# violetamenendez/zest-nerf

Hardware: AMD Instinct MI355X
Metric: rendered rays/sec (1024-ray x 128-sample batch per GPU) (higher is better)
Workload: dtype bf16; 1 GPU; nsff_static_1024x128; rays_per_gpu=1024, samples_per_ray=128, rays_total=1024, collective=none, ranks=1, backend=none

## Files before the change

### zest-nerf_amd/build_hip.py

```python
import os
import subprocess
import sys
from concurrent.futures import ThreadPoolExecutor

HERE = os.path.dirname(os.path.abspath(__file__))
CSRC = os.path.join(HERE, "csrc")
OBJ = os.path.join(CSRC, "build")
LIB = os.path.join(HERE, "libzest_hip.so")
SOURCES = ["capi.hip", "composite.hip", "composite_bwd.hip", "encode.hip", "rays.hip", "volume_cost.hip", "costreg.hip", "losses.hip", "mlp_plan.hip", "mlp.hip", "mlp_engine.hip", "mlp_train.hip", "mlp_train16.hip",
           "mlp_train16_dw.hip", "fused.hip"]
SOURCE_FLAGS = {"mlp_engine.hip": ["-fno-slp-vectorize"], "mlp_train16.hip": ["-fno-slp-vectorize"]}
_SHAPES = [("s4d2", 4, "true", 2, "false"), ("s2d2", 2, "true", 2, "false"), ("s4d0", 4, "true", 0, "false"),
           ("s2d0", 2, "true", 0, "false"), ("s0d0", 0, "true", 0, "false"), ("s4", 4, "false", 0, "false"),
           ("s2", 2, "false", 0, "false"), ("s0", 0, "false", 0, "false"),
           ("s4v", 4, "false", 0, "true"), ("s2v", 2, "false", 0, "true")]
_PRECS = [("x3", "ZEST_PREC_F16X3"), ("bf16", "ZEST_PREC_BF16"), ("f16", "ZEST_PREC_F16")]
VARIANTS = [("fused_%s_%s" % (pt, tag),
             ["-DZEST_V_PTAG=%s" % pt, "-DZEST_V_EP=%s" % ep, "-DZEST_V_TAG=%s" % tag, "-DZEST_V_NTS=%d" % nts,
              "-DZEST_V_DYN=%s" % dyn, "-DZEST_V_NTD=%d" % ntd, "-DZEST_V_V2=%s" % v2] +
             (["-fno-slp-vectorize"] if (nts or ntd) else []) +
             (["-mllvm", "-amdgpu-use-amdgpu-trackers=1"] if ((nts or ntd) and pt != "x3") else []) +
             (["-mllvm", "-amdgpu-sched-strategy=max-ilp"] if tag == "s0" else []))
            for tag, nts, dyn, ntd, v2 in _SHAPES for pt, ep in _PRECS]
HIPCC = os.environ.get("HIPCC", "/opt/rocm/bin/hipcc")
FLAGS = ["-O3", "--offload-arch=gfx950", "-fPIC", "-std=c++17", "-Wall", "-Wno-unused-function",
         "-Wno-inline-asm",
         "-mllvm", "-pragma-unroll-threshold=1000000"]


def _deps():
    hdr = [os.path.join(CSRC, f) for f in os.listdir(CSRC) if f.endswith((".cuh", ".h"))]
    hdr.append(os.path.join(HERE, "..", "include", "zest_render.h"))
    return hdr


def _stale(target, srcs):
    if not os.path.exists(target):
        return True
    t = os.path.getmtime(target)
    return any(os.path.getmtime(s) > t for s in srcs if os.path.exists(s))


def _compile(src, extra, objname=None):
    obj = os.path.join(OBJ, (objname or src.replace(".hip", "")) + ".o")
    path = os.path.join(CSRC, src)
    if _stale(obj, [path] + _deps()):
        cmd = [HIPCC] + FLAGS + extra + ["-Rpass-analysis=kernel-resource-usage", "-c", path, "-o", obj]
        r = subprocess.run(cmd, capture_output=True, text=True)
        if r.returncode != 0:
            raise RuntimeError("hipcc failed for %s:\n%s" % (src, r.stderr[-6000:]))
        remarks = [l for l in r.stderr.splitlines() if "-Rpass-analysis=kernel-resource-usage" in l]
        with open(obj[:-2] + ".remarks", "w") as f:
            f.write("\n".join(remarks) + "\n")
        rest = [l for l in r.stderr.splitlines() if "-Rpass-analysis=kernel-resource-usage" not in l
                and "loop not unrolled" not in l]
        if any(("warning" in l or "error" in l) for l in rest):
            sys.stderr.write("\n".join(rest) + "\n")
    return obj


def build(force=False, extra_flags=(), tag=None, only=None):
    global OBJ, LIB
    if tag:
        OBJ = os.path.join(CSRC, "build_" + tag)
        LIB = os.path.join(HERE, "libzest_hip_%s.so" % tag)
    os.makedirs(OBJ, exist_ok=True)
    every = [(name, "fused_variant.hip", flags) for name, flags in VARIANTS]
    every += [(s.replace(".hip", ""), s, SOURCE_FLAGS.get(s, [])) for s in SOURCES]
    jobs = [j for j in every if not only or j[0] in only or j[1] in only]
    if force:
        for name, _, _ in jobs:
            o = os.path.join(OBJ, name + ".o")
            if os.path.exists(o):
                os.remove(o)
    with ThreadPoolExecutor(max_workers=int(os.environ.get("ZEST_BUILD_JOBS", "8"))) as ex:
        objs = list(ex.map(lambda j: _compile(j[1], j[2] + list(extra_flags), j[0]), jobs))
    default_obj = os.path.join(CSRC, "build")
    objs += [os.path.join(default_obj, j[0] + ".o") for j in every if j not in jobs]
    if _stale(LIB, objs):
        cmd = [HIPCC, "--offload-arch=gfx950", "-shared", "-fPIC", "-o", LIB] + objs + ["-lrocblas"]
        r = subprocess.run(cmd, capture_output=True, text=True)
        if r.returncode != 0:
            raise RuntimeError("link failed:\n" + r.stderr[-4000:])
    return LIB


if __name__ == "__main__":
    argv = sys.argv[1:]
    tag = argv[argv.index("--tag") + 1] if "--tag" in argv else None
    only = argv[argv.index("--only") + 1].split(",") if "--only" in argv else None
    print(build(force="-f" in argv, extra_flags=[a for a in argv if a.startswith("-D")] + [a[7:] for a in argv if a.startswith("--flag=")], tag=tag, only=only))
```

### zest-nerf_amd/csrc/fused.cuh

```cuda
#pragma once
#include "mlp_engine.cuh"
#include "zest_sample_ops.cuh"

namespace zest {

constexpr int kMaxViews = 16;
constexpr int kCamStride = 24;

struct FusedNet {
    const float *bias;
    const uint4 *tiles;
    const float4 *vol;
    const float4 *imgs;
    const float *w2cs, *intr;
    int D, Hv, Wv, V, H, W;
    int head, v2;
};

struct FusedArgs {
    const float *ndc, *pts, *z, *dir;
    int R, S;
    FusedNet st, dy;
    float frame_idx;
    int white_bkgd;
// ... 158 lines not shown
#pragma unroll
        for (int i = 0; i < NK * 8; i++)
            v[i] = __builtin_amdgcn_fractf(ndc[0] * (13.37f + (float)i) + ndc[2] * 7.1f + (float)grp * 0.31f) - 0.25f;
    }
    valid = false;
#endif
    const int rv = feat_volume_round(n.V);
    if (valid) {
        float vv[4] = {0.f, 0.f, 0.f, 0.f};
        if (grp < 2) {
            float fx = zest_unnorm(ndc[0], n.Wv), fy = zest_unnorm(ndc[1], n.Hv), fz = zest_unnorm(ndc[2], n.D);
            fx = fminf(fmaxf(fx, -2.0f), (float)n.Wv + 1.0f);
            fy = fminf(fmaxf(fy, -2.0f), (float)n.Hv + 1.0f);
            fz = fminf(fmaxf(fz, -2.0f), (float)n.D + 1.0f);
            const float x0f = floorf(fx), y0f = floorf(fy), z0f = floorf(fz);
            const float tx = fx - x0f, ty = fy - y0f, tz = fz - z0f;
            const int x0 = (int)x0f, y0 = (int)y0f, z0 = (int)z0f;
            float4 tap[8];
            float wgt[8];
#pragma unroll
            for (int c = 0; c < 8; c++) {
                const int dx = c & 1, dy = (c >> 1) & 1, dz = c >> 2;
                const int xi = x0 + dx, yi = y0 + dy, zi = z0 + dz;
                const bool ok = (unsigned)xi < (unsigned)n.Wv && (unsigned)yi < (unsigned)n.Hv &&
                                (unsigned)zi < (unsigned)n.D;
                const int xc = min(max(xi, 0), n.Wv - 1), yc = min(max(yi, 0), n.Hv - 1),
                          zc = min(max(zi, 0), n.D - 1);
                wgt[c] = ok ? (dx ? tx : 1.0f - tx) * (dy ? ty : 1.0f - ty) * (dz ? tz : 1.0f - tz) : 0.0f;
#ifdef ZEST_EXPERIMENT_TAP_SAME
                tap[c] = n.vol[(((yc * n.Wv + xc) * n.D + zc) & 0) + grp];
#else
                tap[c] = n.vol[2 * ((yc * n.Wv + xc) * n.D + zc) + grp];
#endif
            }
#pragma unroll
            for (int c = 0; c < 8; c++) {
                vv[0] = fmaf(wgt[c], tap[c].x, vv[0]), vv[1] = fmaf(wgt[c], tap[c].y, vv[1]);
                vv[2] = fmaf(wgt[c], tap[c].z, vv[2]), vv[3] = fmaf(wgt[c], tap[c].w, vv[3]);
            }
        }
#pragma unroll
        for (int r = 0; r < 2 * NK; r++) {
            float *dst = v + 8 * (r >> 1) + 4 * (r & 1);
            if (r < rv) {
                view_tap(4 * r + grp, dst);
            } else if (r == rv) {
                if (n.V > 4 * rv) view_tap(grp >= 2 ? 4 * rv + grp - 2 : n.V, dst);
                if (grp < 2) dst[0] = vv[0], dst[1] = vv[1], dst[2] = vv[2], dst[3] = vv[3];
            }
        }
    }
#pragma unroll
    for (int t = 0; t < NK; t++) {
        float w8[8];
#pragma unroll
        for (int e = 0; e < 8; e++) w8[e] = v[8 * t + e];
        store_tile<EP>(w8, op, t);
    }
}

template <bool PROJ>
__device__ __forceinline__ void stage_cams(const FusedNet &n, float *lds) {
    if (!n.w2cs) return;
    const int nv = n.imgs ? n.V : 1;
    for (int i = threadIdx.x; i < nv * kCamStride; i += blockDim.x) {
        const int v = i / kCamStride, k = i % kCamStride;
        float val = 0.0f;
        if constexpr (PROJ) {
            if (k < 12 && n.intr) {
                const int row = k >> 2, col = k & 3;
                const float *K = n.intr + 9 * v + 3 * row, *Rt = n.w2cs + 16 * v + col;
                val = fmaf(K[2], Rt[8], fmaf(K[1], Rt[4], K[0] * Rt[0]));
            } else if (k >= 12) {
                val = n.w2cs[16 * v + (k - 12)];
            }
        } else {
            if (k < 12) val = n.w2cs[16 * v + k];
            else if (k < 21 && n.intr) val = n.intr[9 * v + (k - 12)];
        }
        lds[i] = val;
    }
}

#ifndef ZEST_FUSED_WAVES
#define ZEST_FUSED_WAVES 8
#endif
constexpr int kFusedWaves = ZEST_FUSED_WAVES;
constexpr int kPartialFloats = 20;
constexpr int fused_cb(int EP) { return EP == ZEST_PREC_F16X3 ? 1 : 2; }

struct BlockSamples {
    float x[4], pw[3], zz, dist;
    bool valid;
};

template <int BS>
__device__ __forceinline__ float block_sum(float v) {
    if constexpr (BS == 32) return lower_half_sum(v);
    v += dpp_f<0xB1>(0.f, v);
    v += dpp_f<0x4E>(0.f, v);
    v += dpp_f<0x141>(0.f, v);
    v += dpp_f<0x140>(0.f, v);
    return readlane_f<0>(v);
}
template <int BS>
__device__ __forceinline__ float block_excl_prod(float f, int c, float *total) {
    if constexpr (BS == 32) return lower_half_excl_prod(f, c, total);
    float v = f;
    v *= dpp_f<0x111>(1.f, v);
    v *= dpp_f<0x112>(1.f, v);
    v *= dpp_f<0x114>(1.f, v);
    v *= dpp_f<0x118>(1.f, v);
    *total = readlane_f<15>(v);
    const float ex = dpp_f<0x138>(1.f, v);
    return c == 0 ? 1.0f : ex;
}

#ifndef ZEST_FUSED_WG_PER_CU
#define ZEST_FUSED_WG_PER_CU 1
#endif
#ifndef ZEST_REBUILD_PTS
#define ZEST_REBUILD_PTS 0
#endif
#ifndef ZEST_GATHER_FENCE
#define ZEST_GATHER_FENCE 1
#endif
#ifndef ZEST_EARLY_DYN_GATHER
#define ZEST_EARLY_DYN_GATHER 0
#endif
template <int EP, int NT_FEAT_S, bool DYN, int NT_FEAT_D, bool V2S = false>
__global__ __launch_bounds__(kFusedWaves * 64, kFusedWaves * ZEST_FUSED_WG_PER_CU / 4) void fused_blocks_kernel(FusedArgs a) {
    constexpr bool MOD_S = NT_FEAT_S > 0, MOD_D = NT_FEAT_D > 0;
    constexpr int NP = ep_parts(EP), CB = fused_cb(EP), BS = 16 * CB;
    if constexpr (EP == ZEST_PREC_F16) engine_fp16_overflow_clamp();
    constexpr int UNITS_S = stream_units(4, NT_FEAT_S, NP), UNITS_D = DYN ? stream_units(6, NT_FEAT_D, NP) : 0;
    using Ring = RingTiles<kFusedWaves, UNITS_S, UNITS_D>;
    constexpr int kFdBytes = (DYN && MOD_D && ZEST_EARLY_DYN_GATHER) ? kFusedWaves * CB * (NT_FEAT_D / 2) * NP * 1024 : 0;
    constexpr int kStBytes = DYN ? kFusedWaves * 32 * 24 : 0;
    constexpr bool kMc = mcache_for(EP, MOD_S, NT_FEAT_S / 2) || (DYN && mcache_for(EP, MOD_D, NT_FEAT_D / 2));
    constexpr int kMcWaveBytes = kMc ? kMcJB * CB * 1024 : 0;
    __shared__ __attribute__((aligned(16))) char lds[kRingUnits * 1024 + 2 * kMaxViews * kCamStride * 4 +
                                                     kFusedWaves * 32 * 8 + 2 * kSlots * 4 +
                                                     kFusedWaves * kPartialFloats * 4 + kFusedWaves * 32 * 16 +
                                                     kFdBytes + kStBytes + 2 * kCarryFloats * 4 +
                                                     kFusedWaves * kMcWaveBytes];
    static_assert(sizeof(lds) <= 163840, "LDS budget of one workgroup per CU");
    static_assert((sizeof(lds) - kFusedWaves * kMcWaveBytes) % 16 == 0, "the modulation cache starts 16-byte aligned");
    float *cams_s = reinterpret_cast<float *>(lds + kRingUnits * 1024), *cams_d = cams_s + kMaxViews * kCamStride;
    float2 *zd_lds = reinterpret_cast<float2 *>(cams_d + kMaxViews * kCamStride);
    constexpr bool PROJ = EP != ZEST_PREC_F16X3;
    stage_cams<PROJ>(a.st, cams_s);
    if (DYN) stage_cams<PROJ>(a.dy, cams_d);
    int *ring_flags = reinterpret_cast<int *>(zd_lds + kFusedWaves * 32);
    float *rec_lds = reinterpret_cast<float *>(ring_flags + 2 * kSlots);
    float4 *x_lds = reinterpret_cast<float4 *>(rec_lds + kFusedWaves * kPartialFloats);
    uint4 *fd_lds = reinterpret_cast<uint4 *>(x_lds + kFusedWaves * 32);
    float2 *st_lds = reinterpret_cast<float2 *>(reinterpret_cast<char *>(fd_lds) + kFdBytes);
    float *carry_lds = reinterpret_cast<float *>(reinterpret_cast<char *>(st_lds) + kStBytes);
    char *mc_lds = lds + sizeof(lds) - kFusedWaves * kMcWaveBytes;
#ifdef ZEST_RING_FLAGS
    Ring::init_flags(ring_flags);
#endif
    __syncthreads();

    const int lane0 = threadIdx.x & 63;
    const int wave = __builtin_amdgcn_readfirstlane(threadIdx.x >> 6);
    const Ring tiles{lds, (gptr_u4)a.st.tiles, (gptr_u4)a.dy.tiles, lane0, lane0 >> 4, wave,
                     (unsigned)(wave * Ring::kPieces * 64 + lane0) * 16u,
                     (unsigned)(uintptr_t)(__attribute__((address_space(3))) char *)lds +
                         (unsigned)wave * Ring::kPieces * 1024u
#ifdef ZEST_RING_FLAGS
                     , (unsigned)(uintptr_t)(__attribute__((address_space(3))) char *)ring_flags
#endif
    };
    tiles.init_addr();
    if constexpr (kMc)
        tiles.init_mcache((unsigned)(uintptr_t)(__attribute__((address_space(3))) char *)mc_lds +
                          (unsigned)wave * kMcWaveBytes + (unsigned)lane0 * 16u);
    tiles.prologue();

    const bool ranges = a.ray_ranges != 0;
    const int n_wg = (int)gridDim.x;
#ifndef ZEST_NO_XCD_ORDER
    const int wg = n_wg % 8 == 0 ? (int)(blockIdx.x % 8) * (n_wg / 8) + (int)(blockIdx.x / 8) : (int)blockIdx.x;
#else
    const int wg = (int)blockIdx.x;
#endif
    int range_b0, range_nb;
    if (ranges) {
        range_b0 = (int)((long long)wg * a.R / n_wg) * a.bpr;
        range_nb = (int)((long long)(wg + 1) * a.R / n_wg) * a.bpr - range_b0;
    } else {
        const int n_blocks = a.R * a.bpr;
        const int share = ((n_blocks + kFusedWaves - 1) / kFusedWaves + n_wg - 1) / n_wg * kFusedWaves;
        range_b0 = wg * share, range_nb = min(share, n_blocks - range_b0);
    }
    auto block_of = [&](int pass) {
        const int lb = pass * kFusedWaves + wave;
        return __builtin_amdgcn_readfirstlane(lb < range_nb ? range_b0 + lb : -1);
    };
    auto fetch = [&](int g, int cb, int col, BlockSamples &b) {
        const int r = g >= 0 ? g / a.bpr : 0, s = (g >= 0 ? g % a.bpr : 0) * BS + 16 * cb + col;
        b.valid = g >= 0 && s < a.S;
        b.x[0] = b.x[1] = b.x[2] = 0.f, b.x[3] = a.frame_idx;
        b.pw[0] = b.pw[1] = b.pw[2] = 0.f, b.zz = 0.f, b.dist = 0.f;
        const float *dir = a.dir + 3 * r;
        if (b.valid) {
            const size_t m = (size_t)r * a.S + s;
            const float *zr = a.z + (size_t)r * a.S;
            b.x[0] = a.ndc[3 * m], b.x[1] = a.ndc[3 * m + 1], b.x[2] = a.ndc[3 * m + 2];
            if (a.pts) b.pw[0] = a.pts[3 * m], b.pw[1] = a.pts[3 * m + 1], b.pw[2] = a.pts[3 * m + 2];
            b.zz = zr[s];
            const float dnorm = sqrtf(dir[0] * dir[0] + dir[1] * dir[1] + dir[2] * dir[2]);
            b.dist = ((s + 1 < a.S) ? (zr[s + 1] - b.zz) : 1e10f) * dnorm;
        }
    };
    auto join = [](const f32x4 (&t)[CB], int i) {
        if constexpr (CB == 1) {
            return t[0][i];
        } else {
            const auto r = __builtin_amdgcn_permlane16_swap(__float_as_uint(t[0][i]), __float_as_uint(t[CB - 1][i]), false, false);
            return __uint_as_float(r[0]);
        }
    };
#ifdef ZEST_STAMPS
    unsigned long long st_enc = 0, st_eng = 0, st_comp = 0, st_n = 0;
    const unsigned long long st_t0 = __builtin_amdgcn_s_memtime(), st_r0 = __builtin_amdgcn_s_memrealtime();
#define ZEST_STAMP(var) do { const unsigned long long t_ = __builtin_amdgcn_s_memtime(); var += t_ - st_last; st_last = t_; } while (0)
#else
#define ZEST_STAMP(var) do {} while (0)
#endif
    for (int k = 0; k * kFusedWaves < range_nb; k++) {
        const int pass = k;
#ifdef ZEST_STAMPS
        unsigned long long st_last = __builtin_amdgcn_s_memtime();
        st_n++;
#endif
        const int g = block_of(pass);
        if (__builtin_expect(g < 0, 0)) {
            tiles.finish(0, UNITS_S + UNITS_D);
        } else {
        int lane = lane0;
        asm volatile("" : "+v"(lane));
        const int col = lane & 15, grp = lane >> 4, cbs = lane & (BS - 1);
        int unit = 0;
        f32x4 head_s[CB], rgb_s[CB], head_d[CB], rgb_d[CB];
        auto views_of = [&](const FusedNet &n, const float *cams) {
            return [&, cams](OpArr<1, NP> (&views)[CB]) {
                const float *dir = a.dir + 3 * (g >= 0 ? g / a.bpr : 0);
                float dv[4] = {0.f, 0.f, 0.f, 0.f};
                zest_view_dir(dir, n.w2cs ? cams + (PROJ ? 12 : 0) : nullptr, dv);
                encode_pe_operand<EP, 3, 4, 1>(dv, grp, views[0]);
#pragma unroll
                for (int cb = 1; cb < CB; cb++) views[cb] = views[0];
            };
        };
        OpArr<NT_FEAT_S / 2, NP> feat_s[CB];
#pragma unroll
        for (int cb = 0; cb < CB; cb++) {
            BlockSamples b;
            fetch(g, cb, col, b);
            if (grp == 0) {
                zd_lds[wave * 32 + 16 * cb + col] = make_float2(b.zz, b.valid ? b.dist : -1.0f);
                x_lds[wave * 32 + 16 * cb + col] = make_float4(b.x[0], b.x[1], b.x[2], 0.0f);
            }
            if constexpr (MOD_S) encode_feat_operand<EP, NT_FEAT_S / 2>(a.st, cams_s, b.x, b.pw, grp, b.valid, feat_s[cb]);
#if ZEST_GATHER_FENCE
            if constexpr (DYN && NT_FEAT_S >= 4) __builtin_amdgcn_sched_barrier(0);
#endif
            if constexpr (DYN && MOD_D && ZEST_EARLY_DYN_GATHER) {
                OpArr<NT_FEAT_D / 2, NP> fd;
                encode_feat_operand<EP, NT_FEAT_D / 2>(a.dy, cams_d, b.x, b.pw, grp, b.valid, fd);
#pragma unroll
                for (int t = 0; t < NT_FEAT_D / 2; t++)
#pragma unroll
                    for (int pt = 0; pt < NP; pt++)
                        fd_lds[(((wave * CB + cb) * (NT_FEAT_D / 2) + t) * NP + pt) * 64 + lane] =
                            __builtin_bit_cast(uint4, fd.t[pt][t]);
            }
        }
        auto pts_static = [&](OpArr<2, NP> (&o)[CB], int token) __attribute__((always_inline)) {
#pragma unroll
            for (int cb = 0; cb < CB; cb++) {
                int at = wave * 32 + 16 * cb + col;
                asm volatile("" : "+v"(at) : "v"(token));
                const float4 xv = x_lds[at];
                const float x4[4] = {xv.x, xv.y, xv.z, 0.0f};
#ifdef ZEST_EXPERIMENT_NO_ENCODE
#pragma unroll
                for (int t = 0; t < 2; t++) o[cb].t[0][t] = bf16x8{(short)lane, 1, 2, 3, 4, 5, 6, 7};
#else
                encode_pe_operand<EP, 3, 10, 2>(x4, grp, o[cb]);
#endif
            }
        };
        auto pts_dynamic = [&](OpArr<3, NP> (&o)[CB], int token) __attribute__((always_inline)) {
#pragma unroll
            for (int cb = 0; cb < CB; cb++) {
                int at = wave * 32 + 16 * cb + col;
                asm volatile("" : "+v"(at) : "v"(token));
                const float4 xv = x_lds[at];
                const float x4[4] = {xv.x, xv.y, xv.z, a.frame_idx};
                encode_pe_operand<EP, 4, 10, 3>(x4, grp, o[cb]);
            }
        };
        ZEST_STAMP(st_enc);
        if constexpr (ZEST_REBUILD_PTS) {
            engine_forward<EP, CB, 4, MOD_S, NT_FEAT_S, V2S, true>(tiles, unit, pts_static, feat_s,
                                                        views_of(a.st, cams_s), head_s, rgb_s);
        } else {
            OpArr<2, NP> pts_keep[CB];
            pts_static(pts_keep, 0);
            auto pts_copy = [&](OpArr<2, NP> (&o)[CB], int) __attribute__((always_inline)) {
#pragma unroll
                for (int cb = 0; cb < CB; cb++) o[cb] = pts_keep[cb];
            };
            engine_forward<EP, CB, 4, MOD_S, NT_FEAT_S, V2S, true>(tiles, unit, pts_copy, feat_s,
                                                        views_of(a.st, cams_s), head_s, rgb_s);
        }
        ZEST_STAMP(st_eng);
        float rec[kPartialFloats];
#pragma unroll
        for (int i = 0; i < kPartialFloats; i++) rec[i] = 0.f;
        float zz, dist, cr, cg, cb, al_s;
        bool valid;
        {
            const float2 zd = zd_lds[wave * 32 + cbs];
            zz = zd.x, dist = fmaxf(zd.y, 0.0f), valid = zd.y >= 0.0f;
            float sg = join(head_s, 0);
            cr = join(rgb_s, 0), cg = join(rgb_s, 1), cb = join(rgb_s, 2);
            if (V2S) {
                cr = zest_sigmoid(cr), cg = zest_sigmoid(cg), cb = zest_sigmoid(cb), sg = fmaxf(sg, 0.f);
            }
            cr = zest_sigmoid(cr), cg = zest_sigmoid(cg), cb = zest_sigmoid(cb);
            al_s = valid ? 1.0f - expf(-fmaxf(sg, 0.f) * dist) : 0.0f;
            float tot;
            const float w = al_s * block_excl_prod<BS>(1.0f - al_s + 1e-10f, cbs, &tot);
            rec[0] = tot;
            rec[1] = block_sum<BS>(w * cr), rec[2] = block_sum<BS>(w * cg), rec[3] = block_sum<BS>(w * cb);
            rec[4] = block_sum<BS>(w * zz), rec[5] = block_sum<BS>(w);
        }
        if (DYN) {
            const float blend_s = zest_sigmoid(join(head_s, 1));
            if (lane < BS) {
                st_lds[(wave * 3 + 0) * 32 + lane] = make_float2(cr, cg);
                st_lds[(wave * 3 + 1) * 32 + lane] = make_float2(cb, al_s);
                st_lds[(wave * 3 + 2) * 32 + lane] = make_float2(blend_s, 0.0f);
            }
            OpArr<NT_FEAT_D / 2, NP> feat_d[CB];
            if constexpr (MOD_D && ZEST_EARLY_DYN_GATHER) {
#pragma unroll
                for (int cbi = 0; cbi < CB; cbi++)
#pragma unroll
                    for (int t = 0; t < NT_FEAT_D / 2; t++)
#pragma unroll
                        for (int pt = 0; pt < NP; pt++)
                            feat_d[cbi].t[pt][t] = __builtin_bit_cast(
                                bf16x8, fd_lds[(((wave * CB + cbi) * (NT_FEAT_D / 2) + t) * NP + pt) * 64 + lane]);
            } else if constexpr (MOD_D) {
#pragma unroll
                for (int cbi = 0; cbi < CB; cbi++) {
                    BlockSamples b;
                    fetch(g, cbi, col, b);
                    encode_feat_operand<EP, NT_FEAT_D / 2>(a.dy, cams_d, b.x, b.pw, grp, b.valid, feat_d[cbi]);
                }
            }
            ZEST_STAMP(st_comp);
            if constexpr (ZEST_REBUILD_PTS) {
                engine_forward<EP, CB, 6, MOD_D, NT_FEAT_D, false, true>(tiles, unit, pts_dynamic, feat_d,
                                                            views_of(a.dy, cams_d), head_d, rgb_d);
            } else {
                OpArr<3, NP> pts_keep[CB];
                pts_dynamic(pts_keep, 0);
                auto pts_copy = [&](OpArr<3, NP> (&o)[CB], int) __attribute__((always_inline)) {
#pragma unroll
                    for (int cb = 0; cb < CB; cb++) o[cb] = pts_keep[cb];
                };
                engine_forward<EP, CB, 6, MOD_D, NT_FEAT_D, false, true>(tiles, unit, pts_copy, feat_d,
                                                            views_of(a.dy, cams_d), head_d, rgb_d);
            }
            ZEST_STAMP(st_eng);
            const float2 s0 = st_lds[(wave * 3 + 0) * 32 + cbs], s1 = st_lds[(wave * 3 + 1) * 32 + cbs],
                         s2 = st_lds[(wave * 3 + 2) * 32 + cbs];
            cr = s0.x, cg = s0.y, cb = s1.x, al_s = s1.y;
            const float blend = s2.x;
            const float er = zest_sigmoid(join(rgb_d, 0)), eg = zest_sigmoid(join(rgb_d, 1)),
                        eb = zest_sigmoid(join(rgb_d, 2));
            const float sg_d = join(head_d, 0);
            const float a_fg = valid ? 1.0f - expf(-fmaxf(sg_d, 0.f) * dist) : 0.0f;
            const float a_d = a_fg * blend, a_st = al_s * (1.0f - blend);
            float tot_b, tot_f;
            const float Tb = block_excl_prod<BS>((1.0f - a_d) * (1.0f - a_st) + 1e-10f, cbs, &tot_b);
            const float wf = a_fg * block_excl_prod<BS>(1.0f - a_fg + 1e-10f, cbs, &tot_f);
            const float wd = Tb * a_d, ws = Tb * a_st;
            rec[6] = tot_b;
            rec[7] = block_sum<BS>(wd * er + ws * cr), rec[8] = block_sum<BS>(wd * eg + ws * cg);
            rec[9] = block_sum<BS>(wd * eb + ws * cb), rec[10] = block_sum<BS>((wd + ws) * zz);
            rec[11] = block_sum<BS>(wd);
            rec[12] = tot_f;
            rec[13] = block_sum<BS>(wf * er), rec[14] = block_sum<BS>(wf * eg), rec[15] = block_sum<BS>(wf * eb);
            rec[16] = block_sum<BS>(wf * zz);
        }
        if (lane == 0 && g >= 0) {
            float4 *o = ranges ? reinterpret_cast<float4 *>(rec_lds + wave * kPartialFloats)
                               : reinterpret_cast<float4 *>(a.partials + (size_t)g * kPartialFloats);
#pragma unroll
            for (int i = 0; i < (DYN ? 5 : 2); i++)
                o[i] = make_float4(rec[4 * i], rec[4 * i + 1], rec[4 * i + 2], rec[4 * i + 3]);
        }
        }
#ifdef ZEST_EXPERIMENT_NO_FINISH
        if (false) {
#else
        if (ranges) {
#endif
            __syncthreads();
            const int rb = g >= 0 ? g % a.bpr : 0;
            if (lane0 == 0 && g >= 0 && (wave == 0 || rb == 0)) {
                RayState st;
                if (rb != 0) st.load(carry_lds + ((k + 1) & 1) * kCarryFloats);
                const int n = min(a.bpr - rb, kFusedWaves - wave);
                for (int b = 0; b < n; b++) st.chain(rec_lds + (wave + b) * kPartialFloats, DYN);
                if (rb + n == a.bpr) st.emit(a.white_bkgd, a.out + (size_t)(g / a.bpr) * 16);
                else st.save(carry_lds + (k & 1) * kCarryFloats);
            }
        }
        ZEST_STAMP(st_comp);
        tiles.next_pass();
    }
    tiles.drain();
#ifdef ZEST_RING_FLAGS
    if (tiles.poisoned && lane0 == 0) {
        a.partials[0] = __builtin_nanf("");
    }
#endif
#ifdef ZEST_STAMPS
    if (a.stamps && lane0 == 0) {
        unsigned long long *o = a.stamps + (size_t)(blockIdx.x * kFusedWaves + wave) * 8;
        o[0] = __builtin_amdgcn_s_memtime() - st_t0, o[1] = st_enc, o[2] = st_eng, o[3] = st_comp;
        o[4] = tiles.t_wait, o[5] = tiles.t_issue, o[6] = __builtin_amdgcn_s_memrealtime() - st_r0,
        o[7] = st_n | (tiles.t_vm << 16);
    }
#endif
}

#define ZEST_FUSED_VARIANT(ptag, EP, tag, NTS, DYN, NTD, V2S) ZEST_FUSED_VARIANT_(ptag, EP, tag, NTS, DYN, NTD, V2S)
#define ZEST_FUSED_VARIANT_(ptag, EP, tag, NTS, DYN, NTD, V2S)                                   \
    int fused_launch_##ptag##_##tag(const FusedArgs &a, int blocks, hipStream_t stream) {        \
        hipLaunchKernelGGL((fused_blocks_kernel<EP, NTS, DYN, NTD, V2S>), dim3(blocks),          \
                           dim3(kFusedWaves * 64), 0, stream, a);                                \
        ZEST_RETURN_LAUNCH("zest_render_fused_fwd(" #ptag "_" #tag ")");                         \
    }                                                                                            \
    int fused_units_##ptag##_##tag(int which) {                                                  \
        return which == 0 ? stream_units(4, NTS, ep_parts(EP)) : (DYN ? stream_units(6, NTD, ep_parts(EP)) : 0); \
    }

#define ZEST_FUSED_DECL1(ptag, tag)                                                     \
    int fused_launch_##ptag##_##tag(const FusedArgs &a, int blocks, hipStream_t stream); \
    int fused_units_##ptag##_##tag(int which);
#define ZEST_FUSED_DECL(tag) ZEST_FUSED_DECL1(bf16, tag) ZEST_FUSED_DECL1(f16, tag) ZEST_FUSED_DECL1(x3, tag)
ZEST_FUSED_DECL(s0)
ZEST_FUSED_DECL(s2)
ZEST_FUSED_DECL(s4)
ZEST_FUSED_DECL(s0d0)
ZEST_FUSED_DECL(s2d0)
ZEST_FUSED_DECL(s4d0)
ZEST_FUSED_DECL(s2d2)
ZEST_FUSED_DECL(s4d2)
ZEST_FUSED_DECL(s2v)
ZEST_FUSED_DECL(s4v)

}
```

### zest-nerf_amd/csrc/fused.hip

```cpp
#include <string.h>
#include "fused.cuh"
#include "mlp_plan.h"

namespace zest {

__global__ void fused_combine_kernel(const float *__restrict__ partials, int R, int bpr, int dyn,
                                     int white_bkgd, float *__restrict__ out) {
    const int r = blockIdx.x * blockDim.x + threadIdx.x;
    if (r >= R) return;
    combine_ray([&](int b) { return partials + ((size_t)r * bpr + b) * kPartialFloats; }, bpr, dyn != 0,
                white_bkgd, out + (size_t)r * 16);
}

}

namespace {

bool fill_net(const zest_mlp_desc *d, const void *packed, const zest_view_set *vs, int pts_ch, int precision,
              zest::FusedNet *n, int *nt_feat, int *units, const char **err) {
    memset(n, 0, sizeof(*n));
    if (!d || !packed) return *err = "descriptor and packed weights are required", false;
    if (d->in_ch_pts != pts_ch) return *err = "unexpected in_ch_pts for this slot", false;
    if (d->net_type != 0 && d->net_type != 2) return *err = "net_type must be 0 ('v0') or 2 ('v2')", false;
    zest::MlpPlan plan;
    if (!zest::build_plan(*d, precision, zest::ORDER_ACC, &plan, err, false)) return false;
    n->bias = (const float *)packed;
    n->tiles = (const uint4 *)((const char *)packed + plan.bias_bytes);
    n->head = d->head, n->v2 = d->net_type == 2;
    *nt_feat = d->use_feat ? plan.nt_feat : 0;
    *units = plan.n_tiles;
    if (((uintptr_t)packed & 15) != 0) return *err = "packed weights must be 16-byte aligned", false;
    if (vs) {
        n->w2cs = vs->w2cs, n->intr = vs->intrinsics;
        n->vol = (const float4 *)vs->vol_cl, n->imgs = (const float4 *)vs->imgs_cl;
        n->D = vs->D, n->Hv = vs->Hv, n->Wv = vs->Wv, n->V = vs->V, n->H = vs->H, n->W = vs->W;
    }
    if (d->use_feat) {
        if (!vs || !vs->vol_cl || !vs->imgs_cl || !vs->w2cs || !vs->intrinsics)
            return *err = "a net with features needs volume, images and cameras", false;
        if (vs->D < 1 || vs->Hv < 1 || vs->Wv < 1 || vs->H < 2 || vs->W < 2)
            return *err = "bad volume / image shape", false;
        if ((long long)vs->D * vs->Hv * vs->Wv >= (1LL << 30))
            return *err = "volume too large for the fused kernel's 32-bit voxel indices (2^30 voxels)", false;
        if (vs->V < 1 || vs->V > zest::kMaxViews || 8 + 4 * vs->V != d->in_ch_feat)
            return *err = "view count does not match in_ch_feat = 8 + 4V", false;
        if (((uintptr_t)vs->vol_cl | (uintptr_t)vs->imgs_cl) & 15)
            return *err = "volume / images must be 16-byte aligned", false;
    } else {
        n->vol = nullptr, n->imgs = nullptr;
    }
    return true;
}

}

#ifdef ZEST_STAMPS
constexpr size_t kStampBytes = 1024 * 8 * 8 * 8;
#else
constexpr size_t kStampBytes = 0;
#endif

static int g_pass_shape = 0;

extern "C" int zest_render_fused_set_passes(int shape) {
    ZEST_CHECK_ARG(shape >= 0 && shape <= 2,
                   "zest_render_fused_set_passes: shape must be 0 (auto), 1 (dense: equal block shares) or 2 (ray ranges)");
    g_pass_shape = shape;
    return 0;
}

extern "C" int zest_render_fused_pass_shape(int R, int S, int precision, int cus, int *ray_ranges, int *n_wg,
                                            int *rounds) {
    ZEST_CHECK_ARG(R >= 0 && S >= 1 && zest::prec_is_engine(precision) && ray_ranges,
                   "zest_render_fused_pass_shape: bad argument");
    if (cus <= 0) {
        int dev = 0;
        if (hipGetDevice(&dev) != hipSuccess ||
            hipDeviceGetAttribute(&cus, hipDeviceAttributeMultiprocessorCount, dev) != hipSuccess)
            cus = 256;
    }
    const int bs = 16 * zest::fused_cb(precision), bpr = (S + bs - 1) / bs;
    const int W = zest::kFusedWaves;
    const int P = zest_div_up((long long)R * bpr, W), G0 = P < cus ? P : cus;
    const int dense_rounds = G0 ? zest_div_up(P, G0) : 0, dense_wg = G0 ? zest_div_up(P, dense_rounds) : 0;
    const int n = R < cus ? R : cus;
    const int range_rounds = n ? zest_div_up((long long)zest_div_up(R, n) * bpr, W) : 0;
    int take = range_rounds <= dense_rounds ? 1 : 0;
    if (g_pass_shape == 1) take = 0;
    if (g_pass_shape == 2) take = 1;
    *ray_ranges = take;
    if (n_wg) *n_wg = take ? n : dense_wg;
    if (rounds) *rounds = take ? range_rounds : dense_rounds;
    return 0;
}

extern "C" size_t zest_render_fused_workspace(int R, int S) {
    if (R <= 0 || S <= 0) return 16 + kStampBytes;
    return (size_t)R * ((S + 15) / 16) * zest::kPartialFloats * sizeof(float) + kStampBytes;
}

extern "C" int zest_render_fused_fwd(const float *ndc, const float *pts, const float *z,
                                     const float *rays_dir, int R, int S,
                                     const zest_mlp_desc *desc_static, const void *packed_static,
                                     const zest_view_set *views_static,
                                     const zest_mlp_desc *desc_dynamic, const void *packed_dynamic,
                                     const zest_view_set *views_dynamic, float frame_idx,
                                     int precision, int white_bkgd, void *workspace, float *out,
                                     void *stream) {
    if (R == 0) return 0;
    ZEST_CHECK_ARG(ndc && z && rays_dir && out && workspace,
                   "zest_render_fused_fwd: ndc, z, rays_dir, workspace, out required");
    ZEST_CHECK_ARG(((uintptr_t)workspace & 15) == 0, "zest_render_fused_fwd: workspace must be 16-byte aligned");
    ZEST_CHECK_ARG(R >= 0 && S >= 1, "zest_render_fused_fwd: bad shape R=%d S=%d", R, S);
    ZEST_CHECK_ARG(zest::prec_is_engine(precision),
                   "zest_render_fused_fwd: precision must be ZEST_PREC_BF16, _F16 or _F16X3 (the exact-product "
                   "fp32 kernel exists per operator only: zest_mlp_fwd)");
    ZEST_CHECK_ARG(((uintptr_t)out & 15) == 0, "zest_render_fused_fwd: out must be 16-byte aligned");
    zest::FusedArgs a;
    memset(&a, 0, sizeof(a));
    a.ndc = ndc, a.pts = pts, a.z = z, a.dir = rays_dir, a.R = R, a.S = S;
    a.frame_idx = frame_idx, a.white_bkgd = white_bkgd, a.out = out;
    const int bs = 16 * zest::fused_cb(precision);
    a.bpr = (S + bs - 1) / bs, a.partials = (float *)workspace;
#ifdef ZEST_STAMPS
    a.stamps = (unsigned long long *)((char *)workspace + zest_render_fused_workspace(R, S) - kStampBytes);
#endif
    const char *err = nullptr;
    int nts = 0, ntd = 0, units_s = 0, units_d = 0;
    ZEST_CHECK_ARG(fill_net(desc_static, packed_static, views_static, 63, precision, &a.st, &nts, &units_s, &err),
                   "zest_render_fused_fwd: static net: %s", err);
    const bool dyn = desc_dynamic != nullptr;
    if (dyn) {
        ZEST_CHECK_ARG(fill_net(desc_dynamic, packed_dynamic, views_dynamic, 84, precision, &a.dy, &ntd, &units_d, &err),
                       "zest_render_fused_fwd: dynamic net: %s", err);
        ZEST_CHECK_ARG(desc_static->head == ZEST_HEAD_BLEND && desc_dynamic->head == ZEST_HEAD_DYNAMIC,
                       "zest_render_fused_fwd: blending needs a static net with the blend head and "
                       "a dynamic net with the scene-flow heads");
    }
    ZEST_CHECK_ARG(pts || (!a.st.vol && !a.dy.vol), "zest_render_fused_fwd: pts required with features");
    if (R == 0) return 0;
    int dev = 0, cus = 256;
    if (hipGetDevice(&dev) != hipSuccess ||
        hipDeviceGetAttribute(&cus, hipDeviceAttributeMultiprocessorCount, dev) != hipSuccess)
        cus = 256;
    int blocks = 0;
    zest_render_fused_pass_shape(R, S, precision, cus, &a.ray_ranges, &blocks, nullptr);
    hipStream_t st = (hipStream_t)stream;
    const bool v2s = a.st.v2 != 0;
    ZEST_CHECK_ARG(!(v2s && (dyn || nts == 0)),
                   "zest_render_fused_fwd: a 'v2' net is rendered by the single-net kernels with features only");
    const int key = (v2s ? 1000 : 0) + (dyn ? 100 : 0) + nts * 10 + ntd;
    int rc = -1;
#define ZEST_CASE1(ptag, tag)                                                                    \
    ZEST_CHECK_ARG(zest::fused_units_##ptag##_##tag(0) == units_s && zest::fused_units_##ptag##_##tag(1) == units_d, \
                   "zest_render_fused_fwd: packed stream is %d+%d units, kernel expects %d+%d",  \
                   units_s, units_d, zest::fused_units_##ptag##_##tag(0), zest::fused_units_##ptag##_##tag(1)); \
    rc = zest::fused_launch_##ptag##_##tag(a, blocks, st);
#define ZEST_CASE(k, tag)                                                                        \
    case k:                                                                                      \
        if (precision == ZEST_PREC_BF16) { ZEST_CASE1(bf16, tag) }                               \
        else if (precision == ZEST_PREC_F16) { ZEST_CASE1(f16, tag) }                            \
        else { ZEST_CASE1(x3, tag) }                                                             \
        break;
    switch (key) {
        ZEST_CASE(0, s0)
// ... 22 lines not shown
```

### zest-nerf_amd/csrc/fused_variant.hip

```cpp
#include "fused.cuh"
namespace zest {
ZEST_FUSED_VARIANT(ZEST_V_PTAG, ZEST_V_EP, ZEST_V_TAG, ZEST_V_NTS, ZEST_V_DYN, ZEST_V_NTD, ZEST_V_V2)
}
```

Before: 9.526 million rays/s.

## Run static-only fused kernel with four waves each handling two blocks per pass

Decouples the number of blocks processed per pass from the number of waves, so that the static-only (s0) bf16/f16 variants launch four-wave workgroups in which each wave handles two sample blocks per pass. Per-block state (z, dist, validity, partial records, ray chaining) becomes arrays indexed by the per-wave block slot. The s0 variants also build with an MFMA VGPR-form compiler flag. The goal is more per-wave ILP and MFMA work per instruction stream and fewer waves contending for the CU. The cost is higher register pressure per wave and less latency hiding across waves.

```diff
diff --git a/zest-nerf_amd/build_hip.py b/zest-nerf_amd/build_hip.py
--- a/zest-nerf_amd/build_hip.py
+++ b/zest-nerf_amd/build_hip.py
@@ -20,7 +20,8 @@
               "-DZEST_V_DYN=%s" % dyn, "-DZEST_V_NTD=%d" % ntd, "-DZEST_V_V2=%s" % v2] +
              (["-fno-slp-vectorize"] if (nts or ntd) else []) +
              (["-mllvm", "-amdgpu-use-amdgpu-trackers=1"] if ((nts or ntd) and pt != "x3") else []) +
-             (["-mllvm", "-amdgpu-sched-strategy=max-ilp"] if tag == "s0" else []))
+             (["-mllvm", "-amdgpu-sched-strategy=max-ilp"] if tag == "s0" else []) +
+             (["-DZEST_V_WAVES=4", "-mllvm", "-amdgpu-mfma-vgpr-form"] if (tag == "s0" and pt != "x3") else []))
             for tag, nts, dyn, ntd, v2 in _SHAPES for pt, ep in _PRECS]
 HIPCC = os.environ.get("HIPCC", "/opt/rocm/bin/hipcc")
 FLAGS = ["-O3", "--offload-arch=gfx950", "-fPIC", "-std=c++17", "-Wall", "-Wno-unused-function",
diff --git a/zest-nerf_amd/csrc/fused.cuh b/zest-nerf_amd/csrc/fused.cuh
--- a/zest-nerf_amd/csrc/fused.cuh
+++ b/zest-nerf_amd/csrc/fused.cuh
@@ -264,10 +264,7 @@
     }
 }
 
-#ifndef ZEST_FUSED_WAVES
-#define ZEST_FUSED_WAVES 8
-#endif
-constexpr int kFusedWaves = ZEST_FUSED_WAVES;
+constexpr int kPassBlocks = 8;
 constexpr int kPartialFloats = 20;
 constexpr int fused_cb(int EP) { return EP == ZEST_PREC_F16X3 ? 1 : 2; }
 
@@ -310,36 +307,37 @@
 #ifndef ZEST_EARLY_DYN_GATHER
 #define ZEST_EARLY_DYN_GATHER 0
 #endif
-template <int EP, int NT_FEAT_S, bool DYN, int NT_FEAT_D, bool V2S = false>
-__global__ __launch_bounds__(kFusedWaves * 64, kFusedWaves * ZEST_FUSED_WG_PER_CU / 4) void fused_blocks_kernel(FusedArgs a) {
+template <int EP, int NT_FEAT_S, bool DYN, int NT_FEAT_D, bool V2S = false, int NW = 8>
+__global__ __launch_bounds__(NW * 64, NW * ZEST_FUSED_WG_PER_CU / 4) void fused_blocks_kernel(FusedArgs a) {
     constexpr bool MOD_S = NT_FEAT_S > 0, MOD_D = NT_FEAT_D > 0;
-    constexpr int NP = ep_parts(EP), CB = fused_cb(EP), BS = 16 * CB;
+    static_assert(NW == 8 || NW == 4, "waves per workgroup");
+    constexpr int NP = ep_parts(EP), CBB = fused_cb(EP), BS = 16 * CBB, BPW = kPassBlocks / NW, CB = CBB * BPW;
     if constexpr (EP == ZEST_PREC_F16) engine_fp16_overflow_clamp();
     constexpr int UNITS_S = stream_units(4, NT_FEAT_S, NP), UNITS_D = DYN ? stream_units(6, NT_FEAT_D, NP) : 0;
-    using Ring = RingTiles<kFusedWaves, UNITS_S, UNITS_D>;
-    constexpr int kFdBytes = (DYN && MOD_D && ZEST_EARLY_DYN_GATHER) ? kFusedWaves * CB * (NT_FEAT_D / 2) * NP * 1024 : 0;
-    constexpr int kStBytes = DYN ? kFusedWaves * 32 * 24 : 0;
+    using Ring = RingTiles<NW, UNITS_S, UNITS_D>;
+    constexpr int kFdBytes = (DYN && MOD_D && ZEST_EARLY_DYN_GATHER) ? kPassBlocks * CBB * (NT_FEAT_D / 2) * NP * 1024 : 0;
+    constexpr int kStBytes = DYN ? kPassBlocks * 32 * 24 : 0;
     constexpr bool kMc = mcache_for(EP, MOD_S, NT_FEAT_S / 2) || (DYN && mcache_for(EP, MOD_D, NT_FEAT_D / 2));
     constexpr int kMcWaveBytes = kMc ? kMcJB * CB * 1024 : 0;
     __shared__ __attribute__((aligned(16))) char lds[kRingUnits * 1024 + 2 * kMaxViews * kCamStride * 4 +
-                                                     kFusedWaves * 32 * 8 + 2 * kSlots * 4 +
-                                                     kFusedWaves * kPartialFloats * 4 + kFusedWaves * 32 * 16 +
+                                                     kPassBlocks * 32 * 8 + 2 * kSlots * 4 +
+                                                     kPassBlocks * kPartialFloats * 4 + kPassBlocks * 32 * 16 +
                                                      kFdBytes + kStBytes + 2 * kCarryFloats * 4 +
-                                                     kFusedWaves * kMcWaveBytes];
+                                                     NW * kMcWaveBytes];
     static_assert(sizeof(lds) <= 163840, "LDS budget of one workgroup per CU");
-    static_assert((sizeof(lds) - kFusedWaves * kMcWaveBytes) % 16 == 0, "the modulation cache starts 16-byte aligned");
+    static_assert((sizeof(lds) - NW * kMcWaveBytes) % 16 == 0, "the modulation cache starts 16-byte aligned");
     float *cams_s = reinterpret_cast<float *>(lds + kRingUnits * 1024), *cams_d = cams_s + kMaxViews * kCamStride;
     float2 *zd_lds = reinterpret_cast<float2 *>(cams_d + kMaxViews * kCamStride);
     constexpr bool PROJ = EP != ZEST_PREC_F16X3;
     stage_cams<PROJ>(a.st, cams_s);
     if (DYN) stage_cams<PROJ>(a.dy, cams_d);
-    int *ring_flags = reinterpret_cast<int *>(zd_lds + kFusedWaves * 32);
+    int *ring_flags = reinterpret_cast<int *>(zd_lds + kPassBlocks * 32);
     float *rec_lds = reinterpret_cast<float *>(ring_flags + 2 * kSlots);
-    float4 *x_lds = reinterpret_cast<float4 *>(rec_lds + kFusedWaves * kPartialFloats);
-    uint4 *fd_lds = reinterpret_cast<uint4 *>(x_lds + kFusedWaves * 32);
+    float4 *x_lds = reinterpret_cast<float4 *>(rec_lds + kPassBlocks * kPartialFloats);
+    uint4 *fd_lds = reinterpret_cast<uint4 *>(x_lds + kPassBlocks * 32);
     float2 *st_lds = reinterpret_cast<float2 *>(reinterpret_cast<char *>(fd_lds) + kFdBytes);
     float *carry_lds = reinterpret_cast<float *>(reinterpret_cast<char *>(st_lds) + kStBytes);
-    char *mc_lds = lds + sizeof(lds) - kFusedWaves * kMcWaveBytes;
+    char *mc_lds = lds + sizeof(lds) - NW * kMcWaveBytes;
 #ifdef ZEST_RING_FLAGS
     Ring::init_flags(ring_flags);
 #endif
@@ -374,11 +372,11 @@
         range_nb = (int)((long long)(wg + 1) * a.R / n_wg) * a.bpr - range_b0;
     } else {
         const int n_blocks = a.R * a.bpr;
-        const int share = ((n_blocks + kFusedWaves - 1) / kFusedWaves + n_wg - 1) / n_wg * kFusedWaves;
+        const int share = ((n_blocks + kPassBlocks - 1) / kPassBlocks + n_wg - 1) / n_wg * kPassBlocks;
         range_b0 = wg * share, range_nb = min(share, n_blocks - range_b0);
     }
-    auto block_of = [&](int pass) {
-        const int lb = pass * kFusedWaves + wave;
+    auto block_of = [&](int pass, int slot) {
+        const int lb = pass * kPassBlocks + slot;
         return __builtin_amdgcn_readfirstlane(lb < range_nb ? range_b0 + lb : -1);
     };
     auto fetch = [&](int g, int cb, int col, BlockSamples &b) {
@@ -397,11 +395,12 @@
             b.dist = ((s + 1 < a.S) ? (zr[s + 1] - b.zz) : 1e10f) * dnorm;
         }
     };
-    auto join = [](const f32x4 (&t)[CB], int i) {
-        if constexpr (CB == 1) {
-            return t[0][i];
+    auto join = [](const f32x4 (&t)[CB], int j, int i) {
+        if constexpr (CBB == 1) {
+            return t[j][i];
         } else {
-            const auto r = __builtin_amdgcn_permlane16_swap(__float_as_uint(t[0][i]), __float_as_uint(t[CB - 1][i]), false, false);
+            const auto r = __builtin_amdgcn_permlane16_swap(__float_as_uint(t[CBB * j][i]), __float_as_uint(t[CBB * j + CBB - 1][i]),
+                                                            false, false);
             return __uint_as_float(r[0]);
         }
     };
@@ -412,14 +411,16 @@
 #else
 #define ZEST_STAMP(var) do {} while (0)
 #endif
-    for (int k = 0; k * kFusedWaves < range_nb; k++) {
+    for (int k = 0; k * kPassBlocks < range_nb; k++) {
         const int pass = k;
 #ifdef ZEST_STAMPS
         unsigned long long st_last = __builtin_amdgcn_s_memtime();
         st_n++;
 #endif
-        const int g = block_of(pass);
-        if (__builtin_expect(g < 0, 0)) {
+        int gs[BPW];
+#pragma unroll
+        for (int j = 0; j < BPW; j++) gs[j] = block_of(pass, wave + NW * j);
+        if (__builtin_expect(gs[0] < 0, 0)) {
             tiles.finish(0, UNITS_S + UNITS_D);
         } else {
         int lane = lane0;
@@ -429,22 +430,26 @@
         f32x4 head_s[CB], rgb_s[CB], head_d[CB], rgb_d[CB];
         auto views_of = [&](const FusedNet &n, const float *cams) {
             return [&, cams](OpArr<1, NP> (&views)[CB]) {
-                const float *dir = a.dir + 3 * (g >= 0 ? g / a.bpr : 0);
-                float dv[4] = {0.f, 0.f, 0.f, 0.f};
-                zest_view_dir(dir, n.w2cs ? cams + (PROJ ? 12 : 0) : nullptr, dv);
-                encode_pe_operand<EP, 3, 4, 1>(dv, grp, views[0]);
-#pragma unroll
-                for (int cb = 1; cb < CB; cb++) views[cb] = views[0];
+#pragma unroll
+                for (int j = 0; j < BPW; j++) {
+                    const float *dir = a.dir + 3 * (gs[j] >= 0 ? gs[j] / a.bpr : 0);
+                    float dv[4] = {0.f, 0.f, 0.f, 0.f};
+                    zest_view_dir(dir, n.w2cs ? cams + (PROJ ? 12 : 0) : nullptr, dv);
+                    encode_pe_operand<EP, 3, 4, 1>(dv, grp, views[CBB * j]);
+#pragma unroll
+                    for (int cb = 1; cb < CBB; cb++) views[CBB * j + cb] = views[CBB * j];
+                }
             };
         };
         OpArr<NT_FEAT_S / 2, NP> feat_s[CB];
 #pragma unroll
         for (int cb = 0; cb < CB; cb++) {
+            const int slot = wave + NW * (cb / CBB), cbb = cb % CBB;
             BlockSamples b;
-            fetch(g, cb, col, b);
+            fetch(gs[cb / CBB], cbb, col, b);
             if (grp == 0) {
-                zd_lds[wave * 32 + 16 * cb + col] = make_float2(b.zz, b.valid ? b.dist : -1.0f);
-                x_lds[wave * 32 + 16 * cb + col] = make_float4(b.x[0], b.x[1], b.x[2], 0.0f);
+                zd_lds[slot * 32 + 16 * cbb + col] = make_float2(b.zz, b.valid ? b.dist : -1.0f);
+                x_lds[slot * 32 + 16 * cbb + col] = make_float4(b.x[0], b.x[1], b.x[2], 0.0f);
             }
             if constexpr (MOD_S) encode_feat_operand<EP, NT_FEAT_S / 2>(a.st, cams_s, b.x, b.pw, grp, b.valid, feat_s[cb]);
 #if ZEST_GATHER_FENCE
@@ -457,14 +462,14 @@
                 for (int t = 0; t < NT_FEAT_D / 2; t++)
 #pragma unroll
                     for (int pt = 0; pt < NP; pt++)
-                        fd_lds[(((wave * CB + cb) * (NT_FEAT_D / 2) + t) * NP + pt) * 64 + lane] =
+                        fd_lds[(((slot * CBB + cbb) * (NT_FEAT_D / 2) + t) * NP + pt) * 64 + lane] =
                             __builtin_bit_cast(uint4, fd.t[pt][t]);
             }
         }
         auto pts_static = [&](OpArr<2, NP> (&o)[CB], int token) __attribute__((always_inline)) {
 #pragma unroll
             for (int cb = 0; cb < CB; cb++) {
-                int at = wave * 32 + 16 * cb + col;
+                int at = (wave + NW * (cb / CBB)) * 32 + 16 * (cb % CBB) + col;
                 asm volatile("" : "+v"(at) : "v"(token));
                 const float4 xv = x_lds[at];
                 const float x4[4] = {xv.x, xv.y, xv.z, 0.0f};
@@ -479,7 +484,7 @@
         auto pts_dynamic = [&](OpArr<3, NP> (&o)[CB], int token) __attribute__((always_inline)) {
 #pragma unroll
             for (int cb = 0; cb < CB; cb++) {
-                int at = wave * 32 + 16 * cb + col;
+                int at = (wave + NW * (cb / CBB)) * 32 + 16 * (cb % CBB) + col;
                 asm volatile("" : "+v"(at) : "v"(token));
                 const float4 xv = x_lds[at];
                 const float x4[4] = {xv.x, xv.y, xv.z, a.frame_idx};
@@ -501,34 +506,39 @@
                                                         views_of(a.st, cams_s), head_s, rgb_s);
         }
         ZEST_STAMP(st_eng);
-        float rec[kPartialFloats];
-#pragma unroll
-        for (int i = 0; i < kPartialFloats; i++) rec[i] = 0.f;
-        float zz, dist, cr, cg, cb, al_s;
-        bool valid;
-        {
-            const float2 zd = zd_lds[wave * 32 + cbs];
-            zz = zd.x, dist = fmaxf(zd.y, 0.0f), valid = zd.y >= 0.0f;
-            float sg = join(head_s, 0);
-            cr = join(rgb_s, 0), cg = join(rgb_s, 1), cb = join(rgb_s, 2);
+        float rec[BPW][kPartialFloats];
+        float zz[BPW], dist[BPW];
+        bool valid[BPW];
+#pragma unroll
+        for (int j = 0; j < BPW; j++) {
+            const int slot = wave + NW * j;
+#pragma unroll
+            for (int i = 0; i < kPartialFloats; i++) rec[j][i] = 0.f;
+            float cr, cg, cb, al_s;
+            const float2 zd = zd_lds[slot * 32 + cbs];
+            zz[j] = zd.x, dist[j] = fmaxf(zd.y, 0.0f), valid[j] = zd.y >= 0.0f;
+            float sg = join(head_s, j, 0);
+            cr = join(rgb_s, j, 0), cg = join(rgb_s, j, 1), cb = join(rgb_s, j, 2);
             if (V2S) {
                 cr = zest_sigmoid(cr), cg = zest_sigmoid(cg), cb = zest_sigmoid(cb), sg = fmaxf(sg, 0.f);
             }
             cr = zest_sigmoid(cr), cg = zest_sigmoid(cg), cb = zest_sigmoid(cb);
-            al_s = valid ? 1.0f - expf(-fmaxf(sg, 0.f) * dist) : 0.0f;
+            al_s = valid[j] ? 1.0f - expf(-fmaxf(sg, 0.f) * dist[j]) : 0.0f;
             float tot;
             const float w = al_s * block_excl_prod<BS>(1.0f - al_s + 1e-10f, cbs, &tot);
-            rec[0] = tot;
-            rec[1] = block_sum<BS>(w * cr), rec[2] = block_sum<BS>(w * cg), rec[3] = block_sum<BS>(w * cb);
-            rec[4] = block_sum<BS>(w * zz), rec[5] = block_sum<BS>(w);
+            rec[j][0] = tot;
+            rec[j][1] = block_sum<BS>(w * cr), rec[j][2] = block_sum<BS>(w * cg), rec[j][3] = block_sum<BS>(w * cb);
+            rec[j][4] = block_sum<BS>(w * zz[j]), rec[j][5] = block_sum<BS>(w);
+            if (DYN) {
+                const float blend_s = zest_sigmoid(join(head_s, j, 1));
+                if (lane < BS) {
+                    st_lds[(slot * 3 + 0) * 32 + lane] = make_float2(cr, cg);
+                    st_lds[(slot * 3 + 1) * 32 + lane] = make_float2(cb, al_s);
+                    st_lds[(slot * 3 + 2) * 32 + lane] = make_float2(blend_s, 0.0f);
+                }
+            }
         }
         if (DYN) {
-            const float blend_s = zest_sigmoid(join(head_s, 1));
-            if (lane < BS) {
-                st_lds[(wave * 3 + 0) * 32 + lane] = make_float2(cr, cg);
-                st_lds[(wave * 3 + 1) * 32 + lane] = make_float2(cb, al_s);
-                st_lds[(wave * 3 + 2) * 32 + lane] = make_float2(blend_s, 0.0f);
-            }
             OpArr<NT_FEAT_D / 2, NP> feat_d[CB];
             if constexpr (MOD_D && ZEST_EARLY_DYN_GATHER) {
 #pragma unroll
@@ -538,12 +548,12 @@
 #pragma unroll
                         for (int pt = 0; pt < NP; pt++)
                             feat_d[cbi].t[pt][t] = __builtin_bit_cast(
-                                bf16x8, fd_lds[(((wave * CB + cbi) * (NT_FEAT_D / 2) + t) * NP + pt) * 64 + lane]);
+                                bf16x8, fd_lds[((((wave + NW * (cbi / CBB)) * CBB + cbi % CBB) * (NT_FEAT_D / 2) + t) * NP + pt) * 64 + lane]);
             } else if constexpr (MOD_D) {
 #pragma unroll
                 for (int cbi = 0; cbi < CB; cbi++) {
                     BlockSamples b;
-                    fetch(g, cbi, col, b);
+                    fetch(gs[cbi / CBB], cbi % CBB, col, b);
                     encode_feat_operand<EP, NT_FEAT_D / 2>(a.dy, cams_d, b.x, b.pw, grp, b.valid, feat_d[cbi]);
                 }
             }
@@ -562,33 +572,40 @@
                                                             views_of(a.dy, cams_d), head_d, rgb_d);
             }
             ZEST_STAMP(st_eng);
-            const float2 s0 = st_lds[(wave * 3 + 0) * 32 + cbs], s1 = st_lds[(wave * 3 + 1) * 32 + cbs],
-                         s2 = st_lds[(wave * 3 + 2) * 32 + cbs];
-            cr = s0.x, cg = s0.y, cb = s1.x, al_s = s1.y;
-            const float blend = s2.x;
-            const float er = zest_sigmoid(join(rgb_d, 0)), eg = zest_sigmoid(join(rgb_d, 1)),
-                        eb = zest_sigmoid(join(rgb_d, 2));
-            const float sg_d = join(head_d, 0);
-            const float a_fg = valid ? 1.0f - expf(-fmaxf(sg_d, 0.f) * dist) : 0.0f;
-            const float a_d = a_fg * blend, a_st = al_s * (1.0f - blend);
-            float tot_b, tot_f;
-            const float Tb = block_excl_prod<BS>((1.0f - a_d) * (1.0f - a_st) + 1e-10f, cbs, &tot_b);
-            const float wf = a_fg * block_excl_prod<BS>(1.0f - a_fg + 1e-10f, cbs, &tot_f);
-            const float wd = Tb * a_d, ws = Tb * a_st;
-            rec[6] = tot_b;
-            rec[7] = block_sum<BS>(wd * er + ws * cr), rec[8] = block_sum<BS>(wd * eg + ws * cg);
-            rec[9] = block_sum<BS>(wd * eb + ws * cb), rec[10] = block_sum<BS>((wd + ws) * zz);
-            rec[11] = block_sum<BS>(wd);
-            rec[12] = tot_f;
-            rec[13] = block_sum<BS>(wf * er), rec[14] = block_sum<BS>(wf * eg), rec[15] = block_sum<BS>(wf * eb);
-            rec[16] = block_sum<BS>(wf * zz);
-        }
-        if (lane == 0 && g >= 0) {
-            float4 *o = ranges ? reinterpret_cast<float4 *>(rec_lds + wave * kPartialFloats)
-                               : reinterpret_cast<float4 *>(a.partials + (size_t)g * kPartialFloats);
-#pragma unroll
-            for (int i = 0; i < (DYN ? 5 : 2); i++)
-                o[i] = make_float4(rec[4 * i], rec[4 * i + 1], rec[4 * i + 2], rec[4 * i + 3]);
+#pragma unroll
+            for (int j = 0; j < BPW; j++) {
+                const int slot = wave + NW * j;
+                const float2 s0 = st_lds[(slot * 3 + 0) * 32 + cbs], s1 = st_lds[(slot * 3 + 1) * 32 + cbs],
+                             s2 = st_lds[(slot * 3 + 2) * 32 + cbs];
+                const float cr = s0.x, cg = s0.y, cb = s1.x, al_s = s1.y;
+                const float blend = s2.x;
+                const float er = zest_sigmoid(join(rgb_d, j, 0)), eg = zest_sigmoid(join(rgb_d, j, 1)),
+                            eb = zest_sigmoid(join(rgb_d, j, 2));
+                const float sg_d = join(head_d, j, 0);
+                const float a_fg = valid[j] ? 1.0f - expf(-fmaxf(sg_d, 0.f) * dist[j]) : 0.0f;
+                const float a_d = a_fg * blend, a_st = al_s * (1.0f - blend);
+                float tot_b, tot_f;
+                const float Tb = block_excl_prod<BS>((1.0f - a_d) * (1.0f - a_st) + 1e-10f, cbs, &tot_b);
+                const float wf = a_fg * block_excl_prod<BS>(1.0f - a_fg + 1e-10f, cbs, &tot_f);
+                const float wd = Tb * a_d, ws = Tb * a_st;
+                rec[j][6] = tot_b;
+                rec[j][7] = block_sum<BS>(wd * er + ws * cr), rec[j][8] = block_sum<BS>(wd * eg + ws * cg);
+                rec[j][9] = block_sum<BS>(wd * eb + ws * cb), rec[j][10] = block_sum<BS>((wd + ws) * zz[j]);
+                rec[j][11] = block_sum<BS>(wd);
+                rec[j][12] = tot_f;
+                rec[j][13] = block_sum<BS>(wf * er), rec[j][14] = block_sum<BS>(wf * eg), rec[j][15] = block_sum<BS>(wf * eb);
+                rec[j][16] = block_sum<BS>(wf * zz[j]);
+            }
+        }
+#pragma unroll
+        for (int j = 0; j < BPW; j++) {
+            if (lane == 0 && gs[j] >= 0) {
+                float4 *o = ranges ? reinterpret_cast<float4 *>(rec_lds + (wave + NW * j) * kPartialFloats)
+                                   : reinterpret_cast<float4 *>(a.partials + (size_t)gs[j] * kPartialFloats);
+#pragma unroll
+                for (int i = 0; i < (DYN ? 5 : 2); i++)
+                    o[i] = make_float4(rec[j][4 * i], rec[j][4 * i + 1], rec[j][4 * i + 2], rec[j][4 * i + 3]);
+            }
         }
         }
 #ifdef ZEST_EXPERIMENT_NO_FINISH
@@ -597,14 +614,18 @@
         if (ranges) {
 #endif
             __syncthreads();
-            const int rb = g >= 0 ? g % a.bpr : 0;
-            if (lane0 == 0 && g >= 0 && (wave == 0 || rb == 0)) {
-                RayState st;
-                if (rb != 0) st.load(carry_lds + ((k + 1) & 1) * kCarryFloats);
-                const int n = min(a.bpr - rb, kFusedWaves - wave);
-                for (int b = 0; b < n; b++) st.chain(rec_lds + (wave + b) * kPartialFloats, DYN);
-                if (rb + n == a.bpr) st.emit(a.white_bkgd, a.out + (size_t)(g / a.bpr) * 16);
-                else st.save(carry_lds + (k & 1) * kCarryFloats);
+#pragma unroll
+            for (int j = 0; j < BPW; j++) {
+                const int slot = wave + NW * j, g = gs[j];
+                const int rb = g >= 0 ? g % a.bpr : 0;
+                if (lane0 == 0 && g >= 0 && (slot == 0 || rb == 0)) {
+                    RayState st;
+                    if (rb != 0) st.load(carry_lds + ((k + 1) & 1) * kCarryFloats);
+                    const int n = min(a.bpr - rb, kPassBlocks - slot);
+                    for (int b = 0; b < n; b++) st.chain(rec_lds + (slot + b) * kPartialFloats, DYN);
+                    if (rb + n == a.bpr) st.emit(a.white_bkgd, a.out + (size_t)(g / a.bpr) * 16);
+                    else st.save(carry_lds + (k & 1) * kCarryFloats);
+                }
             }
         }
         ZEST_STAMP(st_comp);
@@ -618,7 +639,7 @@
 #endif
 #ifdef ZEST_STAMPS
     if (a.stamps && lane0 == 0) {
-        unsigned long long *o = a.stamps + (size_t)(blockIdx.x * kFusedWaves + wave) * 8;
+        unsigned long long *o = a.stamps + (size_t)(blockIdx.x * NW + wave) * 8;
         o[0] = __builtin_amdgcn_s_memtime() - st_t0, o[1] = st_enc, o[2] = st_eng, o[3] = st_comp;
         o[4] = tiles.t_wait, o[5] = tiles.t_issue, o[6] = __builtin_amdgcn_s_memrealtime() - st_r0,
         o[7] = st_n | (tiles.t_vm << 16);
@@ -626,11 +647,11 @@
 #endif
 }
 
-#define ZEST_FUSED_VARIANT(ptag, EP, tag, NTS, DYN, NTD, V2S) ZEST_FUSED_VARIANT_(ptag, EP, tag, NTS, DYN, NTD, V2S)
-#define ZEST_FUSED_VARIANT_(ptag, EP, tag, NTS, DYN, NTD, V2S)                                   \
+#define ZEST_FUSED_VARIANT(ptag, EP, tag, NTS, DYN, NTD, V2S, NW) ZEST_FUSED_VARIANT_(ptag, EP, tag, NTS, DYN, NTD, V2S, NW)
+#define ZEST_FUSED_VARIANT_(ptag, EP, tag, NTS, DYN, NTD, V2S, NW)                               \
     int fused_launch_##ptag##_##tag(const FusedArgs &a, int blocks, hipStream_t stream) {        \
-        hipLaunchKernelGGL((fused_blocks_kernel<EP, NTS, DYN, NTD, V2S>), dim3(blocks),          \
-                           dim3(kFusedWaves * 64), 0, stream, a);                                \
+        hipLaunchKernelGGL((fused_blocks_kernel<EP, NTS, DYN, NTD, V2S, NW>), dim3(blocks),      \
+                           dim3(NW * 64), 0, stream, a);                                         \
         ZEST_RETURN_LAUNCH("zest_render_fused_fwd(" #ptag "_" #tag ")");                         \
     }                                                                                            \
     int fused_units_##ptag##_##tag(int which) {                                                  \
diff --git a/zest-nerf_amd/csrc/fused.hip b/zest-nerf_amd/csrc/fused.hip
--- a/zest-nerf_amd/csrc/fused.hip
+++ b/zest-nerf_amd/csrc/fused.hip
@@ -80,7 +80,7 @@
             cus = 256;
     }
     const int bs = 16 * zest::fused_cb(precision), bpr = (S + bs - 1) / bs;
-    const int W = zest::kFusedWaves;
+    const int W = zest::kPassBlocks;
     const int P = zest_div_up((long long)R * bpr, W), G0 = P < cus ? P : cus;
     const int dense_rounds = G0 ? zest_div_up(P, G0) : 0, dense_wg = G0 ? zest_div_up(P, dense_rounds) : 0;
     const int n = R < cus ? R : cus;
diff --git a/zest-nerf_amd/csrc/fused_variant.hip b/zest-nerf_amd/csrc/fused_variant.hip
--- a/zest-nerf_amd/csrc/fused_variant.hip
+++ b/zest-nerf_amd/csrc/fused_variant.hip
@@ -1,4 +1,7 @@
 #include "fused.cuh"
+#ifndef ZEST_V_WAVES
+#define ZEST_V_WAVES 8
+#endif
 namespace zest {
-ZEST_FUSED_VARIANT(ZEST_V_PTAG, ZEST_V_EP, ZEST_V_TAG, ZEST_V_NTS, ZEST_V_DYN, ZEST_V_NTD, ZEST_V_V2)
+ZEST_FUSED_VARIANT(ZEST_V_PTAG, ZEST_V_EP, ZEST_V_TAG, ZEST_V_NTS, ZEST_V_DYN, ZEST_V_NTD, ZEST_V_V2, ZEST_V_WAVES)
 }
```

Measured after the change: 9.297 million rays/s (median of 2 runs). 2.4% lower.
